# Golbstein/Keras-segmentation-deeplab-v3.1

Measured on AMD Instinct MI355X. Metric: images/sec fwd+bwd, 512x512 MobileNetV2 OS=16, 21 classes, higher is better.
Workload: dtype f32; 1 GPU; Deeplabv3(backbone='mobilenetv2', input_shape=(512,512,3), classes=21, OS=16) head=deeplab: fwd + sparse-xent loss + bwd + Adam, BN batch mode, dropout 0.1; global_batch=128, per_gpu_batch=128, parallelism=dp1, hipgraph=True, matrix_math=f32, dist_strict=False, backward_fork=False

## Files before the change

### keras-segmentation-deeplab-v3.1_amd/csrc/dwconv.hip

```cpp
#include "common.h"

#pragma clang fp contract(on)
#include <type_traits>
#include <stdlib.h>

namespace {

__device__ __forceinline__ f32x4 ld4_su(const float *base, unsigned byte_off) {
  return ld4(reinterpret_cast<const float *>(reinterpret_cast<const char *>(base) + byte_off));
}
__device__ __forceinline__ void st4_nt_su(float *base, unsigned byte_off, f32x4 v) {
  st4_nt(reinterpret_cast<float *>(reinterpret_cast<char *>(base) + byte_off), v);
}

struct DwGeom {
  int N, H, W, C, stride, rate, pad_t, pad_l, Ho, Wo;
  int prows;
};

struct DwMarch {
  int H, W, C, r, nchunk, TK, nxseg, nphase, ppb, nslab, ny, N;
  int prows;
  int fast;
};
// ... 313 lines not shown
    };
    if (ph.k0 < ph.k1) dw_walk<R>(ph, allact, ph.ke, group);
    if (!ph.bot_halo && ph.k0 < ph.k1) {
      float *orow = yn + (size_t)(a + (ph.k1 - 1) * r) * W * C;
      if (act_a) { st4_nt_su(orow, osa, aA); s1 += aA; s2 += aA * aA; }
      if (act_b) { st4_nt_su(orow, osb, bA); s1 += bA; s2 += bA * bA; }
    }
  }
  dw_store_stats(part, dw_tile_row(M, tile), M.N * M.ny * M.nxseg, M.prows, C, c, s1, s2, red);
}

template <bool SXK, bool ADDK>
__global__ __launch_bounds__(256, 2) void dw_march_bwd(
    const float *__restrict__ g, const float *__restrict__ yraw, const float *__restrict__ cA,
    const float *__restrict__ cB, const float *__restrict__ cC, const float *__restrict__ x,
    const float *__restrict__ sc, const float *__restrict__ sh, int act, const float *__restrict__ w,
    float *__restrict__ dx, const float *__restrict__ dx_add, const float *__restrict__ xmean,
    const float *__restrict__ xinvstd, float *__restrict__ dpart, float *__restrict__ wpart, DwMarch M,
    const float *__restrict__ sx) {
  __shared__ float red[4 * 8 * 36];
  const int tid = threadIdx.x, cq = tid & 7, pl = tid >> 3;
  DwTile tile;
  if (!dw_tile(M, tile)) return;
  const int H = M.H, W = M.W, C = M.C, r = M.r;
  const int xs = tile.xs, slab = tile.slab, n = tile.n;
  const int c = slab * 32 + cq * 4;
  const int xx = xs * 32 + pl;
  const bool active = (c < C) && (xx < W);

  const DwChan cn = dw_chan(c, C, w, sc, sh, cA, cB, cC, dpart != nullptr, xmean, xinvstd);
  const bool xl_ok = (xx - r >= 0), xr_ok = (xx + r < W);
  const int cc = min(c, C - 4), xc = min(xx, W - 1), xlc = min(max(xx - r, 0), W - 1), xrc = min(xx + r, W - 1);
  const size_t nimg = (size_t)n * H * W * C;
  const unsigned om = 4u * (unsigned)(xc * C + cc), ol = 4u * (unsigned)(xlc * C + cc), orr = 4u * (unsigned)(xrc * C + cc);
  const unsigned oo = 4u * (unsigned)(xx * C + c);
  const bool allact = M.fast && (slab * 32 + 32 <= C) && (xs * 32 + 32 <= W);
  f32x4 dwv[9];
#pragma unroll
  for (int i = 0; i < 9; i++) dwv[i] = splat4(0.f);
  f32x4 s1 = splat4(0.f), s2 = splat4(0.f);
  for (int pi = 0; pi < M.ppb; ++pi) {
    DwPhase ph;
    if (!dw_phase(M, tile.pc, pi, ph)) break;
    const int a = ph.a;
    const float *yr = dw_yr(cA, yraw, g);
    auto rowoff = [&](int k) -> size_t { return nimg + (size_t)(a + min(max(k, 0), ph.Kc) * r) * W * C; };

    auto ld_dd1 = [&](size_t row, unsigned off) -> f32x4 { return dw_dy(cn, ld4_su(g + row, off), ld4_su(yr + row, off)); };
    auto ld_dd = [&](int k, f32x4 &l, f32x4 &m, f32x4 &rr) {
      const bool rok = active && k >= 0 && k < ph.Ka;
      const size_t row = rowoff(k);
      const f32x4 vm = ld_dd1(row, om), vl = ld_dd1(row, ol), vr = ld_dd1(row, orr);
      m = vm * splat4(rok ? 1.f : 0.f);
      l = vl * splat4((rok && xl_ok) ? 1.f : 0.f);
      rr = vr * splat4((rok && xr_ok) ? 1.f : 0.f);
    };
    auto ld_e = [&](int k, f32x4 &raw, bool &ok) {
      ok = active && k >= 0 && k < ph.Ka;
      raw = ld4_su(x + rowoff(k), om);
    };
    auto eact = [&](f32x4 raw, bool ok) -> f32x4 {
      const f32x4 v = dl3_act4(cn.s * raw + cn.t, act);
      return v * splat4(ok ? 1.f : 0.f);
    };

    f32x4 accA = splat4(0.f), accB = splat4(0.f);

    if (ph.k0 < ph.k1) {
      constexpr int R = 2;
      f32x4 e_prev = splat4(0.f), e_cur, e_next;
      bool ok_prev = false, ok_cur, ok_next;
      ld_e(ph.ks, e_cur, ok_cur);
      ld_e(ph.ks + 1, e_next, ok_next);
      auto group = [&](int kg, auto fastc) __attribute__((always_inline)) {
        constexpr bool FAST = decltype(fastc)::value, SXC = SXK, ADDC = ADDK;
        f32x4 l[R], m[R], rr[R], e_new[R], sxv[R], addv[R];
        bool ok_new[R];
#pragma unroll
        for (int j = 0; j < R; j++) {
          if constexpr (FAST) {
            const size_t row = nimg + (size_t)(a + (kg + j) * r) * W * C;
            m[j] = ld_dd1(row, om);
            l[j] = ld_dd1(row, ol) * splat4(xl_ok ? 1.f : 0.f);
            rr[j] = ld_dd1(row, orr) * splat4(xr_ok ? 1.f : 0.f);
            ld_e(kg + j + 2, e_new[j], ok_new[j]);
            const size_t orow = nimg + (size_t)(a + (kg + j - 1) * r) * W * C;
            if constexpr (SXC) sxv[j] = ld4_su(sx + orow, om);
            if constexpr (ADDC) addv[j] = ld4_su(dx_add + orow, om);
          } else {
            ld_dd((kg + j <= ph.ke) ? kg + j : -1, l[j], m[j], rr[j]);
            ld_e(kg + j + 2, e_new[j], ok_new[j]);
            const size_t orow = rowoff(kg + j - 1);
            if constexpr (SXC) sxv[j] = ld4_su(sx + orow, om);
            if constexpr (ADDC) addv[j] = ld4_su(dx_add + orow, om);
          }
        }
#pragma unroll
        for (int j = 0; j < R; j++) {
          const int k = kg + j;
          const bool kv = FAST || k <= ph.ke;
          if (FAST || (k >= ph.k0 && k < ph.k1)) {
            f32x4 ea0 = eact(e_prev, ok_prev), ea1 = eact(e_cur, ok_cur), ea2 = eact(e_next, ok_next);
            dwv[0] += ea0 * rr[j]; dwv[1] += ea0 * m[j]; dwv[2] += ea0 * l[j];
            dwv[3] += ea1 * rr[j]; dwv[4] += ea1 * m[j]; dwv[5] += ea1 * l[j];
            dwv[6] += ea2 * rr[j]; dwv[7] += ea2 * m[j]; dwv[8] += ea2 * l[j];
          }
          f32x4 h0 = cn.wv[0] * rr[j] + cn.wv[1] * m[j] + cn.wv[2] * l[j];
          f32x4 h1 = cn.wv[3] * rr[j] + cn.wv[4] * m[j] + cn.wv[5] * l[j];
          f32x4 h2 = cn.wv[6] * rr[j] + cn.wv[7] * m[j] + cn.wv[8] * l[j];
          f32x4 out = accA + h0;
          if constexpr (FAST) {
            out = out * dl3_mask4(cn.s * e_prev + cn.t, act);
            if constexpr (ADDC) out += addv[j];
            st4_nt_su(dx + nimg + (size_t)(a + (k - 1) * r) * W * C, oo, out);
            s1 += out;
            s2 += out * (((SXC ? sxv[j] : e_prev) - cn.mu) * cn.is);
            accA = accB + h1;
            accB = h2;
            e_prev = e_cur; ok_prev = ok_cur;
            e_cur = e_next; ok_cur = ok_next;
            e_next = e_new[j]; ok_next = ok_new[j];
          } else {
            if (dx && active && kv && k - 1 >= ph.k0 && k - 1 < ph.k1) {
              out = out * dl3_mask4(cn.s * e_prev + cn.t, act);
              if constexpr (ADDC) out += addv[j];
              st4_nt_su(dx + nimg + (size_t)(a + (k - 1) * r) * W * C, oo, out);
              s1 += out;
              s2 += out * (((SXC ? sxv[j] : e_prev) - cn.mu) * cn.is);
            }
            accA = kv ? accB + h1 : accA;
            accB = kv ? h2 : accB;
            e_prev = kv ? e_cur : e_prev; ok_prev = kv ? ok_cur : ok_prev;
            e_cur = kv ? e_next : e_cur; ok_cur = kv ? ok_next : ok_cur;
            e_next = kv ? e_new[j] : e_next; ok_next = kv ? ok_new[j] : ok_next;
          }
        }
      };
      dw_walk<R>(ph, allact && dx, ph.k1 - 1, group);
      if (!ph.bot_halo && dx && active) {
        const size_t row = nimg + (size_t)(a + (ph.k1 - 1) * r) * W * C;
        f32x4 out = accA * dl3_mask4(cn.s * e_prev + cn.t, act);
        if constexpr (ADDK) out += ld4_su(dx_add + row, oo);
        st4_nt_su(dx + row, oo, out);
        s1 += out;
        s2 += out * (((SXK ? ld4_su(sx + row, oo) : e_prev) - cn.mu) * cn.is);
      }
    }
  }
  const int p = dw_tile_row(M, tile), written = M.N * M.ny * M.nxseg;
  dw_store_wgrad(wpart, p, written, M.prows, C, c, dwv, red);
  dw_store_stats(dpart, p, written, M.prows, C, c, s1, s2, red);
}

__global__ __launch_bounds__(256) void dw_gather_fwd(const float *__restrict__ x, const float *__restrict__ sc,
                                                     const float *__restrict__ sh, int act,
                                                     const float *__restrict__ w, float *__restrict__ y, DwGeom G,
                                                     float *__restrict__ part) {
  __shared__ float red[4 * 8 * 8];
  const int tid = threadIdx.x, cq = tid & 7, pl = tid >> 3;
  const int c = blockIdx.x * 32 + cq * 4;
  const bool cok = c < G.C;
  const DwChan cn = dw_chan(c, G.C, w, sc, sh);
  f32x4 s1 = splat4(0.f), s2 = splat4(0.f);
  const long NP = (long)G.N * G.Ho * G.Wo;
  for (long p = (long)blockIdx.y * 32 + pl; p < NP && cok; p += (long)gridDim.y * 32) {
    const int ox = (int)(p % G.Wo);
    const int oy = (int)((p / G.Wo) % G.Ho);
    const int n = (int)(p / ((long)G.Wo * G.Ho));
    f32x4 acc = splat4(0.f);
    f32x4 tap[9];
    float okf[9];
#pragma unroll
    for (int i = 0; i < 3; i++) {
      const int iy = oy * G.stride - G.pad_t + i * G.rate;
      const int iyc = min(max(iy, 0), G.H - 1);
#pragma unroll
      for (int j = 0; j < 3; j++) {
        const int ix = ox * G.stride - G.pad_l + j * G.rate;
        const int ixc = min(max(ix, 0), G.W - 1);
        okf[i * 3 + j] = (iy == iyc && ix == ixc) ? 1.f : 0.f;
        tap[i * 3 + j] = ld4(x + (((size_t)n * G.H + iyc) * G.W + ixc) * G.C + c);
      }
    }
#pragma unroll
    for (int q = 0; q < 9; q++) acc += (cn.wv[q] * splat4(okf[q])) * dl3_act4(cn.s * tap[q] + cn.t, act);
    st4_nt(y + (size_t)p * G.C + c, acc);
    s1 += acc;
    s2 += acc * acc;
  }
  dw_store_stats(part, blockIdx.y, gridDim.y, G.prows, G.C, c, s1, s2, red);
}

__global__ __launch_bounds__(256) void dw_gather_bwd(
    const float *__restrict__ g, const float *__restrict__ yraw, const float *__restrict__ cA,
    const float *__restrict__ cB, const float *__restrict__ cC, const float *__restrict__ x,
    const float *__restrict__ sc, const float *__restrict__ sh, int act, const float *__restrict__ w,
    float *__restrict__ dx, const float *__restrict__ dx_add, const float *__restrict__ xmean,
    const float *__restrict__ xinvstd, float *__restrict__ dpart, float *__restrict__ wpart, DwGeom G) {
  __shared__ float red[4 * 8 * 36];
  const int tid = threadIdx.x, cq = tid & 7, pl = tid >> 3;
  const int c = blockIdx.x * 32 + cq * 4;
  const bool cok = c < G.C;
  const DwChan cn = dw_chan(c, G.C, w, sc, sh, cA, cB, cC, dpart != nullptr, xmean, xinvstd);
  f32x4 dwv[9];
#pragma unroll
  for (int i = 0; i < 9; i++) dwv[i] = splat4(0.f);
  f32x4 s1 = splat4(0.f), s2 = splat4(0.f);
  const long NP = (long)G.N * G.H * G.W;
  for (long p = (long)blockIdx.y * 32 + pl; p < NP && cok; p += (long)gridDim.y * 32) {
    const int ix = (int)(p % G.W);
    const int iy = (int)((p / G.W) % G.H);
    const int n = (int)(p / ((long)G.W * G.H));
    const f32x4 eraw = ld4(x + (size_t)p * G.C + c);
    const f32x4 z = cn.s * eraw + cn.t;
    const f32x4 ea = dl3_act4(z, act);
    f32x4 acc = splat4(0.f);
    const float *yr = dw_yr(cA, yraw, g);
    f32x4 tg[9], ty_[9];
    float okf[9];
#pragma unroll
    for (int i = 0; i < 3; i++) {
      const int ty = iy + G.pad_t - i * G.rate;
      const int oy = max(ty, 0) / G.stride;
      const bool yok = ty >= 0 && (ty % G.stride) == 0 && oy < G.Ho;
      const int oyc = min(oy, G.Ho - 1);
#pragma unroll
      for (int j = 0; j < 3; j++) {
        const int tx = ix + G.pad_l - j * G.rate;
        const int ox = max(tx, 0) / G.stride;
        const bool xok = tx >= 0 && (tx % G.stride) == 0 && ox < G.Wo;
        const int oxc = min(ox, G.Wo - 1);
        const size_t off = (((size_t)n * G.Ho + oyc) * G.Wo + oxc) * G.C + c;
        okf[i * 3 + j] = (yok && xok) ? 1.f : 0.f;
        tg[i * 3 + j] = ld4(g + off);
        ty_[i * 3 + j] = ld4(yr + off);
      }
    }
#pragma unroll
    for (int q = 0; q < 9; q++) {
      const f32x4 dd = dw_dy(cn, tg[q], ty_[q]) * splat4(okf[q]);
      acc += dd * cn.wv[q];
      dwv[q] += ea * dd;
    }
    if (dx) {
      f32x4 out = acc * dl3_mask4(z, act);
      if (dx_add) out += ld4(dx_add + (size_t)p * G.C + c);
      st4_nt(dx + (size_t)p * G.C + c, out);
      s1 += out;
      s2 += out * ((eraw - cn.mu) * cn.is);
    }
  }
  dw_store_wgrad(wpart, blockIdx.y, gridDim.y, G.prows, G.C, c, dwv, red);
  dw_store_stats(dpart, blockIdx.y, gridDim.y, G.prows, G.C, c, s1, s2, red);
}

__global__ __launch_bounds__(256) void dw_s2_bwd(
    const float *__restrict__ g, const float *__restrict__ yraw, const float *__restrict__ cA,
    const float *__restrict__ cB, const float *__restrict__ cC, const float *__restrict__ x,
    const float *__restrict__ sc, const float *__restrict__ sh, int act, const float *__restrict__ w,
    float *__restrict__ dx, const float *__restrict__ dx_add, const float *__restrict__ xmean,
    const float *__restrict__ xinvstd, float *__restrict__ dpart, float *__restrict__ wpart, DwGeom G) {
  __shared__ float red[4 * 8 * 36];
  const int tid = threadIdx.x, cq = tid & 7, pl = tid >> 3;
  const int c = blockIdx.x * 32 + cq * 4;
  const bool cok = c < G.C;
  const int cc = min(c, G.C - 4);
  const DwChan cn = dw_chan(c, G.C, w, sc, sh, cA, cB, cC, dpart != nullptr, xmean, xinvstd);
  const float *yr = dw_yr(cA, yraw, g);
  f32x4 dwv[9];
#pragma unroll
  for (int i = 0; i < 9; i++) dwv[i] = splat4(0.f);
  f32x4 s1 = splat4(0.f), s2 = splat4(0.f);
  const int A = (G.H + G.pad_t + 1) / 2, Bn = (G.W + G.pad_l + 1) / 2;
  const long NB = (long)G.N * A * Bn;
  for (long q = (long)blockIdx.y * 32 + pl; q < NB; q += (long)gridDim.y * 32) {
    const int b = (int)(q % Bn), a = (int)((q / Bn) % A), n = (int)(q / ((long)Bn * A));
    const int iy0 = 2 * a - G.pad_t, ix0 = 2 * b - G.pad_l;
    f32x4 dd[2][2];
#pragma unroll
    for (int i = 0; i < 2; i++)
#pragma unroll
      for (int j = 0; j < 2; j++) {
        const int oy = a - i, ox = b - j;
        const int oyc = min(max(oy, 0), G.Ho - 1), oxc = min(max(ox, 0), G.Wo - 1);
        const float ok = (cok && oy == oyc && ox == oxc) ? 1.f : 0.f;
        const size_t off = (((size_t)n * G.Ho + oyc) * G.Wo + oxc) * G.C + cc;
        dd[i][j] = dw_dy(cn, ld4(g + off), ld4(yr + off)) * splat4(ok);
      }
    f32x4 xr[2][2], ad[2][2];
    float pok[2][2];
    size_t poff[2][2];
#pragma unroll
    for (int i = 0; i < 2; i++)
#pragma unroll
      for (int j = 0; j < 2; j++) {
        const int iy = iy0 + i, ix = ix0 + j;
        const int iyc = min(max(iy, 0), G.H - 1), ixc = min(max(ix, 0), G.W - 1);
        pok[i][j] = (cok && iy == iyc && ix == ixc) ? 1.f : 0.f;
        poff[i][j] = (((size_t)n * G.H + iyc) * G.W + ixc) * G.C + cc;
        xr[i][j] = ld4(x + poff[i][j]);
        ad[i][j] = dx_add ? ld4(dx_add + poff[i][j]) : splat4(0.f);
      }
    f32x4 acc[2][2];
    acc[0][0] = cn.wv[0] * dd[0][0] + cn.wv[6] * dd[1][0] + cn.wv[2] * dd[0][1] + cn.wv[8] * dd[1][1];
    acc[0][1] = cn.wv[1] * dd[0][0] + cn.wv[7] * dd[1][0];
    acc[1][0] = cn.wv[3] * dd[0][0] + cn.wv[5] * dd[0][1];
    acc[1][1] = cn.wv[4] * dd[0][0];
    f32x4 ea[2][2];
#pragma unroll
    for (int i = 0; i < 2; i++)
#pragma unroll
      for (int j = 0; j < 2; j++) ea[i][j] = dl3_act4(cn.s * xr[i][j] + cn.t, act) * splat4(pok[i][j]);
    dwv[0] += ea[0][0] * dd[0][0]; dwv[6] += ea[0][0] * dd[1][0]; dwv[2] += ea[0][0] * dd[0][1]; dwv[8] += ea[0][0] * dd[1][1];
    dwv[1] += ea[0][1] * dd[0][0]; dwv[7] += ea[0][1] * dd[1][0];
    dwv[3] += ea[1][0] * dd[0][0]; dwv[5] += ea[1][0] * dd[0][1];
    dwv[4] += ea[1][1] * dd[0][0];
    if (dx) {
#pragma unroll
      for (int i = 0; i < 2; i++)
#pragma unroll
        for (int j = 0; j < 2; j++) {
          f32x4 out = acc[i][j] * dl3_mask4(cn.s * xr[i][j] + cn.t, act) + ad[i][j];
          if (pok[i][j] != 0.f) {
            st4_nt(dx + poff[i][j], out);
            s1 += out;
            s2 += out * ((xr[i][j] - cn.mu) * cn.is);
          }
        }
    }
  }
  dw_store_wgrad(wpart, blockIdx.y, gridDim.y, G.prows, G.C, c, dwv, red);
  dw_store_stats(dpart, blockIdx.y, gridDim.y, G.prows, G.C, c, s1, s2, red);
}

struct DwPlan {
  int impl;
  int nslab, nxseg, nphase, nchunk, TK;
  int ppb, ny;
  int two;
  int PB;
  int P;
};

// ... 188 lines not shown
```

### keras-segmentation-deeplab-v3.1_amd/csrc/pwfused.hip

```cpp
#include <stdlib.h>

#include <type_traits>

#include "common.h"

namespace {

struct FusedArgs {
  const float *x; int ldx; const float *xs, *xt; int x_act;
  const float *g; int ldg; const float *y; int ldy; const float *cA, *cB, *cC;
  const float *wT;
  float *slab;
  float *dx; int lddx;
  const float *add; int ldadd;
  const float *sx; int ldsx; const float *mean, *invstd;
  float *part;
  int M, K, N, Mper;
};

constexpr int FMS = 32;

template <int KB, int NB, bool AUX>
__global__ __launch_bounds__(256, (KB * NB == 5 || AUX) ? 2 : 4) void pw_bwd_fused_kernel(FusedArgs P) {
  constexpr int KP = KB * 32, NP = NB * 32;
  constexpr int LDX = KP + 4, LDD = NP + 4, LDW = KP;
  constexpr int NBLK = KB * NB;
  constexpr int WB = (NBLK + 3) / 4;
  constexpr int XB = (KB + 3) / 4;
  __shared__ float Xr[FMS * LDX];
  __shared__ float Ds[FMS * LDD];
  __shared__ float Sx[AUX ? FMS * LDX : 1];
  __shared__ float Ad[AUX ? FMS * LDX : 1];
  __shared__ float Wl[NP * LDW];
  __shared__ float cfx[2 * KP];
  __shared__ float cfd[3 * NP];

  const int tid = threadIdx.x, lane = tid & 63, wave = tid >> 6;
  const int l31 = lane & 31, lhi = lane >> 5;
  const int bz = blockIdx.x;
  const int mbeg = bz * P.Mper, mend = min(P.M, mbeg + P.Mper);
  const bool two = (P.cA != nullptr);
  const bool sep = AUX && P.sx != nullptr && P.sx != P.x;
  const float hi = (P.x_act == DL3_ACT_RELU6) ? 6.f : __builtin_inff();

  for (int i = tid; i < KP; i += 256) {
    const int k = min(i, P.K - 1);
    cfx[i] = P.xs ? P.xs[k] : 1.f;
    cfx[KP + i] = P.xs ? P.xt[k] : 0.f;
  }
  for (int i = tid; i < NP; i += 256) {
    const int n = min(i, P.N - 1);
    cfd[i] = two ? P.cA[n] : 1.f;
    cfd[NP + i] = two ? P.cB[n] : 0.f;
    cfd[2 * NP + i] = two ? P.cC[n] : 0.f;
  }
  for (int i = tid; i < NP * KP; i += 256) {
    const int n = i / KP, k = i % KP;
    Wl[n * LDW + k] = (n < P.N && k < P.K) ? P.wT[(size_t)n * P.K + k] : 0.f;
  }

  f32x16 accw[WB];
#pragma unroll
  for (int b = 0; b < WB; b++)
#pragma unroll
    for (int r = 0; r < 16; r++) accw[b][r] = 0.f;
  float st1[XB], st2[XB];
#pragma unroll
  for (int b = 0; b < XB; b++) st1[b] = st2[b] = 0.f;

  f32x4 rx[KB], rg[NB], ry[NB], rs[AUX ? KB : 1], ra[AUX ? KB : 1];
  auto load_regs = [&](int m0) {
#pragma unroll
    for (int i = 0; i < KB; i++) {
      const int idx = tid + 256 * i;
      const int mr = idx / (KP / 4), kq = idx % (KP / 4);
      const int row = min(m0 + mr, P.M - 1), k = min(kq * 4, P.K - 4);
      rx[i] = ld4(P.x + (size_t)row * P.ldx + k);
      if constexpr (AUX) {
        if (sep) rs[i] = ld4(P.sx + (size_t)row * P.ldsx + k);
        if (P.add) ra[i] = ld4(P.add + (size_t)row * P.ldadd + k);
      }
    }
#pragma unroll
    for (int i = 0; i < NB; i++) {
      const int idx = tid + 256 * i;
      const int mr = idx / (NP / 4), nq = idx % (NP / 4);
      const int row = min(m0 + mr, P.M - 1), n = min(nq * 4, P.N - 4);
      rg[i] = ld4(P.g + (size_t)row * P.ldg + n);
      if (two) ry[i] = ld4(P.y + (size_t)row * P.ldy + n);
    }
  };
  auto store_lds = [&](int m0) {
#pragma unroll
    for (int i = 0; i < KB; i++) {
      const int idx = tid + 256 * i;
      const int mr = idx / (KP / 4), kq = idx % (KP / 4);
      st4(&Xr[mr * LDX + kq * 4], rx[i]);
      if constexpr (AUX) {
        if (sep) st4(&Sx[mr * LDX + kq * 4], rs[i]);
        if (P.add) st4(&Ad[mr * LDX + kq * 4], ra[i]);
      }
    }
#pragma unroll
    for (int i = 0; i < NB; i++) {
      const int idx = tid + 256 * i;
      const int mr = idx / (NP / 4), nq = idx % (NP / 4);
      const bool ok = (m0 + mr) < mend && nq * 4 < P.N;
      f32x4 v = ld4(cfd + nq * 4) * rg[i] + ld4(cfd + 2 * NP + nq * 4);
      if (two) v += ld4(cfd + NP + nq * 4) * ry[i];
      if (!ok) v = splat4(0.f);
      st4(&Ds[mr * LDD + nq * 4], v);
    }
  };

  __syncthreads();
  if (mbeg < mend) load_regs(mbeg);
  for (int m0 = mbeg; m0 < mend; m0 += FMS) {
    store_lds(m0);
    __syncthreads();
    if (m0 + FMS < mend) load_regs(m0 + FMS);

#pragma unroll
    for (int b = 0; b < WB; b++) {
      const int blk = wave + 4 * b;
      if (blk < NBLK) {
        const int kb = blk / NB, nb = blk % NB;
        const float sk = cfx[kb * 32 + l31], tk = cfx[KP + kb * 32 + l31];
#pragma unroll
        for (int s = 0; s < FMS / 2; s++) {
          const float a = dl3_act(sk * Xr[(2 * s + lhi) * LDX + kb * 32 + l31] + tk, P.x_act);
          const float bb = Ds[(2 * s + lhi) * LDD + nb * 32 + l31];
          accw[b] = __builtin_amdgcn_mfma_f32_32x32x2f32(a, bb, accw[b], 0, 0, 0);
        }
      }
    }
#pragma unroll
    for (int kx = 0; kx < XB; kx++) {
      const int kbx = 4 * kx + (3 - wave);
      if (kbx < KB) {
        f32x16 acc;
#pragma unroll
        for (int r = 0; r < 16; r++) acc[r] = 0.f;
#pragma unroll 8
        for (int s = 0; s < NP / 2; s++) {
          const float a = Ds[l31 * LDD + 2 * s + lhi];
          const float bb = Wl[(2 * s + lhi) * LDW + kbx * 32 + l31];
          acc = __builtin_amdgcn_mfma_f32_32x32x2f32(a, bb, acc, 0, 0, 0);
        }
        const int col = kbx * 32 + l31;
        const bool cok = col < P.K;
        const float sc = cfx[col], tc = cfx[KP + col];
        const float mu = (P.part && cok) ? P.mean[col] : 0.f, is = (P.part && cok) ? P.invstd[col] : 0.f;
#pragma unroll
        for (int r = 0; r < 16; r++) {
          const int rl = (r & 3) + 8 * (r >> 2) + 4 * lhi;
          const int row = m0 + rl;
          const float raw = Xr[rl * LDX + col];
          float v = acc[r];
          if (P.x_act != DL3_ACT_NONE) {
            const float z = sc * raw + tc;
            v = (z > 0.f && z < hi) ? v : 0.f;
          }
          float xh = raw;
          if constexpr (AUX) {
            if (P.add) v += Ad[rl * LDX + col];
            if (sep) xh = Sx[rl * LDX + col];
          }
          if (cok && row < mend) {
            __builtin_nontemporal_store(v, &P.dx[(size_t)row * P.lddx + col]);
            st1[kx] += v;
            st2[kx] += v * ((xh - mu) * is);
          }
        }
// ... 12 lines not shown
#pragma unroll
      for (int r = 0; r < 16; r++) {
        const int krow = kb * 32 + (r & 3) + 8 * (r >> 2) + 4 * lhi;
        if (krow < P.K && col < P.N) out[(size_t)krow * P.N + col] = accw[b][r];
      }
    }
  }
  if (P.part) {
#pragma unroll
    for (int kx = 0; kx < XB; kx++) {
      const int kbx = 4 * kx + (3 - wave);
      if (kbx < KB) {
        const float a1 = st1[kx] + __shfl_xor(st1[kx], 32, 64), a2 = st2[kx] + __shfl_xor(st2[kx], 32, 64);
        const int col = kbx * 32 + l31;
        if (lhi == 0 && col < P.K) {
          P.part[((size_t)bz * P.K + col) * 2 + 0] = a1;
          P.part[((size_t)bz * P.K + col) * 2 + 1] = a2;
        }
      }
    }
  }
}


struct FusedSlices { int lo[4], n[4], maxn; };

constexpr int fused_dw_blocks(int nblk, int w) { return nblk > w ? (nblk - w + 3) / 4 : 0; }

constexpr FusedSlices fused_slices(int KB, int NB) {
  FusedSlices s{};
  const int nblk = KB * NB, TS = 16 * NB, split = 4 / KB;
  int load[4] = {0, 0, 0, 0};
  for (int w = 0; w < 4; w++) { load[w] = 16 * fused_dw_blocks(nblk, w); s.n[w] = 0; s.lo[w] = 0; }
  for (int g = 0; g < KB; g++) {
    for (int t = 0; t < TS; t++) {
      int best = g;
      for (int p = 1; p < split; p++) {
        const int w = g + KB * p;
        if (load[w] <= load[best]) best = w;
      }
      s.n[best]++;
      load[best]++;
    }
    int lo = 0;
    for (int p = 0; p < split; p++) {
      const int w = g + KB * p;
      s.lo[w] = lo;
      lo += s.n[w];
    }
  }
  s.maxn = 0;
  for (int w = 0; w < 4; w++) s.maxn = s.n[w] > s.maxn ? s.n[w] : s.maxn;
  return s;
}

constexpr int cmax(int a, int b) { return a > b ? a : b; }

template <int KB, int NB, bool AUX>
struct Fused2 {
  static constexpr int KP = KB * 32, NP = NB * 32;
  static constexpr int LDX = KP + 4, LDD = NP + 4;
  static constexpr int NBLK = KB * NB;
  static constexpr int WB = (NBLK + 3) / 4;
  static constexpr int SPLIT = KB <= 2 ? 4 / KB : 1;
  static constexpr int XB = SPLIT > 1 ? 1 : (KB + 3) / 4;
  static constexpr int RPW = 16 / SPLIT;
  static constexpr FusedSlices SL = fused_slices(KB <= 2 ? KB : 1, NB);
  static constexpr int NWB = SPLIT > 1 ? SL.maxn : 1;
  static constexpr int LDW = KP;
  static constexpr int O_X = 0;
  static constexpr int O_D = O_X + FMS * LDX;
  static constexpr int O_S = O_D + FMS * LDD;
  static constexpr int O_A = O_S + (AUX ? FMS * LDX : 0);
  static constexpr int O_W = O_A + (AUX ? FMS * LDX : 0);
  static constexpr int O_CX = O_W + (SPLIT > 1 ? 0 : NP * LDW);
  static constexpr int O_CD = O_CX + 2 * KP;
  static constexpr int O_P = O_CD + 3 * NP;
  static constexpr int O_R = O_P + (SPLIT > 1 ? 4 * 1024 : 0);
  static constexpr int TOTAL = O_R + (SPLIT > 1 ? 256 : 0);
};

template <int KB, int NB, bool AUX, int OC>
__global__ __launch_bounds__(256, OC) void pw_bwd_fused2_kernel(FusedArgs P) {
  using C = Fused2<KB, NB, AUX>;
  constexpr int KP = C::KP, NP = C::NP, LDX = C::LDX, LDD = C::LDD, LDW = C::LDW, NBLK = C::NBLK;
  constexpr int SPLIT = C::SPLIT, XB = C::XB, WB = C::WB, NWB = C::NWB;
  __shared__ float smem[C::TOTAL];
  float *const Xr = smem + C::O_X, *const Ds = smem + C::O_D, *const Sx = smem + C::O_S, *const Ad = smem + C::O_A;
  float *const Wl = smem + C::O_W, *const cfx = smem + C::O_CX, *const cfd = smem + C::O_CD;
  float *const Pp = smem + C::O_P, *const red = smem + C::O_R;

  const int tid = threadIdx.x, lane = tid & 63;
  const int wave = __builtin_amdgcn_readfirstlane(tid >> 6);
  const int l31 = lane & 31, lhi = lane >> 5;
  const int bz = blockIdx.x;
  const int mbeg = bz * P.Mper, mend = min(P.M, mbeg + P.Mper);
  const bool two = (P.cA != nullptr);
  const bool sep = AUX && P.sx != nullptr && P.sx != P.x;
  const float hi = (P.x_act == DL3_ACT_RELU6) ? 6.f : __builtin_inff();

  for (int i = tid; i < KP; i += 256) {
    const int k = min(i, P.K - 1);
    cfx[i] = P.xs ? P.xs[k] : 1.f;
    cfx[KP + i] = P.xs ? P.xt[k] : 0.f;
  }
  for (int i = tid; i < NP; i += 256) {
    const int n = min(i, P.N - 1);
    cfd[i] = two ? P.cA[n] : 1.f;
    cfd[NP + i] = two ? P.cB[n] : 0.f;
    cfd[2 * NP + i] = two ? P.cC[n] : 0.f;
  }

  const int klast = P.K - 32 * (KB - 1);
  int x_kbx[XB], x_col[XB], x_lo = 0, x_n = NP / 2, x_part = 0;
  if constexpr (SPLIT > 1) {
    x_kbx[0] = wave % KB;
    x_part = wave / KB;
    x_lo = wave == 0 ? C::SL.lo[0] : wave == 1 ? C::SL.lo[1] : wave == 2 ? C::SL.lo[2] : C::SL.lo[3];
    x_n = wave == 0 ? C::SL.n[0] : wave == 1 ? C::SL.n[1] : wave == 2 ? C::SL.n[2] : C::SL.n[3];
  } else {
#pragma unroll
    for (int kx = 0; kx < XB; kx++) x_kbx[kx] = 4 * kx + (3 - wave);
  }
#pragma unroll
  for (int kx = 0; kx < XB; kx++) x_col[kx] = x_kbx[kx] * 32 + (x_kbx[kx] == KB - 1 ? l31 % klast : l31);
  float x_sc[XB], x_tc[XB], x_mu[XB], x_is[XB];
  float wb[NWB];
  if constexpr (SPLIT > 1) {
#pragma unroll
    for (int s = 0; s < NWB; s++) {
      const int n = 2 * (x_lo + s) + lhi;
      const bool ok = s < x_n && n < P.N;
      const float v = P.wT[(size_t)min(n, P.N - 1) * P.K + x_col[0]];
      wb[s] = ok ? v : 0.f;
    }
  } else {
    wb[0] = 0.f;
    for (int i = tid; i < NP * KP; i += 256) {
      const int n = i / KP, k = i % KP;
      Wl[n * LDW + k] = (n < P.N && k < P.K) ? P.wT[(size_t)n * P.K + k] : 0.f;
    }
  }

  f32x16 accw[WB];
#pragma unroll
  for (int b = 0; b < WB; b++)
#pragma unroll
    for (int r = 0; r < 16; r++) accw[b][r] = 0.f;
  float st1[XB], st2[XB];
#pragma unroll
  for (int b = 0; b < XB; b++) st1[b] = st2[b] = 0.f;

  f32x4 rx[KB], rg[NB], ry[NB], rs[AUX ? KB : 1], ra[AUX ? KB : 1];
  auto load_regs = [&](int m0) {
#pragma unroll
    for (int i = 0; i < KB; i++) {
      const int idx = tid + 256 * i;
      const int mr = idx / (KP / 4), kq = idx % (KP / 4);
      const int row = min(m0 + mr, P.M - 1), k = min(kq * 4, P.K - 4);
      rx[i] = ld4(P.x + (size_t)row * P.ldx + k);
      if constexpr (AUX) {
        if (sep) rs[i] = ld4(P.sx + (size_t)row * P.ldsx + k);
        if (P.add) ra[i] = ld4(P.add + (size_t)row * P.ldadd + k);
      }
    }
#pragma unroll
    for (int i = 0; i < NB; i++) {
      const int idx = tid + 256 * i;
      const int mr = idx / (NP / 4), nq = idx % (NP / 4);
      const int row = min(m0 + mr, P.M - 1), n = min(nq * 4, P.N - 4);
      rg[i] = ld4(P.g + (size_t)row * P.ldg + n);
      if (two) ry[i] = ld4(P.y + (size_t)row * P.ldy + n);
    }
  };
  auto store_lds = [&](int m0) {
#pragma unroll
    for (int i = 0; i < KB; i++) {
      const int idx = tid + 256 * i;
      const int mr = idx / (KP / 4), kq = idx % (KP / 4);
      st4(&Xr[mr * LDX + kq * 4], rx[i]);
      if constexpr (AUX) {
        if (sep) st4(&Sx[mr * LDX + kq * 4], rs[i]);
        if (P.add) st4(&Ad[mr * LDX + kq * 4], ra[i]);
      }
    }
#pragma unroll
    for (int i = 0; i < NB; i++) {
      const int idx = tid + 256 * i;
      const int mr = idx / (NP / 4), nq = idx % (NP / 4);
      const bool ok = (m0 + mr) < mend && nq * 4 < P.N;
      f32x4 v = ld4(cfd + nq * 4) * rg[i] + ld4(cfd + 2 * NP + nq * 4);
      if (two) v += ld4(cfd + NP + nq * 4) * ry[i];
      if (!ok) v = splat4(0.f);
      st4(&Ds[mr * LDD + nq * 4], v);
    }
  };

  auto finish = [&](auto fullc, float v, int m0, int rl, int col, bool own, float sc, float tc, float mu, float is,
                    float &s1, float &s2) {
    constexpr bool FULL = decltype(fullc)::value;
    const int row = m0 + rl;
    const float raw = Xr[rl * LDX + col];
    if (P.x_act != DL3_ACT_NONE) {
      const float z = sc * raw + tc;
      v = (z > 0.f && z < hi) ? v : 0.f;
    }
    float xh = raw;
    if constexpr (AUX) {
      if (P.add) v += Ad[rl * LDX + col];
      if (sep) xh = Sx[rl * LDX + col];
    }
    if constexpr (FULL) {
      __builtin_nontemporal_store(v, &P.dx[(size_t)row * P.lddx + col]);
      s1 += own ? v : 0.f;
      s2 += own ? v * ((xh - mu) * is) : 0.f;
    } else {
      if (own && row < mend) {
        __builtin_nontemporal_store(v, &P.dx[(size_t)row * P.lddx + col]);
        s1 += v;
        s2 += v * ((xh - mu) * is);
      }
    }
  };

  auto stage = [&](auto fullc, int m0) {
#pragma unroll
    for (int b = 0; b < WB; b++) {
      const int blk = wave + 4 * b;
      if (blk < NBLK) {
        const int kb = blk / NB, nb = blk % NB;
        const float sk = cfx[kb * 32 + l31], tk = cfx[KP + kb * 32 + l31];
#pragma unroll 4
        for (int s = 0; s < FMS / 2; s++) {
          const float a = dl3_act(sk * Xr[(2 * s + lhi) * LDX + kb * 32 + l31] + tk, P.x_act);
          const float bb = Ds[(2 * s + lhi) * LDD + nb * 32 + l31];
          accw[b] = __builtin_amdgcn_mfma_f32_32x32x2f32(a, bb, accw[b], 0, 0, 0);
        }
      }
    }

    if constexpr (SPLIT > 1) {
      f32x16 acc;
#pragma unroll
      for (int r = 0; r < 16; r++) acc[r] = 0.f;
      const float *dq = Ds + l31 * LDD + 2 * x_lo + lhi;
#pragma unroll
      for (int s = 0; s < NWB; s++)
        if (s < x_n) acc = __builtin_amdgcn_mfma_f32_32x32x2f32(dq[2 * s], wb[s], acc, 0, 0, 0);
      float *pp = Pp + wave * 1024 + lane;
#pragma unroll
      for (int r = 0; r < 16; r++) pp[r * 64] = acc[r];
      __syncthreads();
      const int kbx = x_kbx[0], col = x_col[0];
      const float *pq = Pp + kbx * 1024 + lane;
      const bool own = kbx * 32 + l31 < P.K;
      const float sc = x_sc[0], tc = x_tc[0], mu = x_mu[0], is = x_is[0];
#pragma unroll
      for (int rr = 0; rr < C::RPW; rr++) {
        const int r = x_part * C::RPW + rr;
        float v = pq[r * 64];
#pragma unroll
        for (int p = 1; p < SPLIT; p++) v += pq[p * KB * 1024 + r * 64];
        finish(fullc, v, m0, (r & 3) + 8 * (r >> 2) + 4 * lhi, col, own, sc, tc, mu, is, st1[0], st2[0]);
      }
    } else {
#pragma unroll
      for (int kx = 0; kx < XB; kx++) {
        const int kbx = x_kbx[kx];
        if (kbx < KB) {
          f32x16 acc;
#pragma unroll
          for (int r = 0; r < 16; r++) acc[r] = 0.f;
          const int col = x_col[kx];
#pragma unroll 8
          for (int s = 0; s < NP / 2; s++) {
            const float a = Ds[l31 * LDD + 2 * s + lhi];
            const float bb = Wl[(2 * s + lhi) * LDW + col];
            acc = __builtin_amdgcn_mfma_f32_32x32x2f32(a, bb, acc, 0, 0, 0);
          }
          const bool own = kbx * 32 + l31 < P.K;
          const float sc = x_sc[kx], tc = x_tc[kx], mu = x_mu[kx], is = x_is[kx];
#pragma unroll
          for (int r = 0; r < 16; r++)
            finish(fullc, acc[r], m0, (r & 3) + 8 * (r >> 2) + 4 * lhi, col, own, sc, tc, mu, is, st1[kx], st2[kx]);
        }
      }
    }
  };

  __syncthreads();
#pragma unroll
  for (int kx = 0; kx < XB; kx++) {
    const int col = min(x_col[kx], KP - 1);
    x_sc[kx] = cfx[col];
    x_tc[kx] = cfx[KP + col];
    x_mu[kx] = P.part ? P.mean[min(col, P.K - 1)] : 0.f;
    x_is[kx] = P.part ? P.invstd[min(col, P.K - 1)] : 0.f;
  }
  const int mfull = mbeg + ((mend > mbeg ? mend - mbeg : 0) / FMS) * FMS;
  if (mbeg < mend) load_regs(mbeg);
  auto whole_stage = [&](int m0) {
    store_lds(m0);
    __syncthreads();
    if (m0 + FMS < mend) load_regs(m0 + FMS);
    stage(std::true_type{}, m0);
    __syncthreads();
  };
  for (int m0 = mbeg; m0 < mfull; m0 += FMS) whole_stage(m0);
  if (mfull < mend) {
    store_lds(mfull);
    __syncthreads();
    stage(std::false_type{}, mfull);
    __syncthreads();
  }

  float *out = P.slab + (size_t)bz * P.K * P.N;
#pragma unroll
  for (int b = 0; b < WB; b++) {
    const int blk = wave + 4 * b;
    if (blk < NBLK) {
      const int kb = blk / NB, nb = blk % NB;
      const int col = nb * 32 + l31;
#pragma unroll
      for (int r = 0; r < 16; r++) {
        const int krow = kb * 32 + (r & 3) + 8 * (r >> 2) + 4 * lhi;
        if (krow < P.K && col < P.N) out[(size_t)krow * P.N + col] = accw[b][r];
      }
    }
  }
  if (P.part) {
    if constexpr (SPLIT > 1) {
      const float a1 = st1[0] + __shfl_xor(st1[0], 32, 64), a2 = st2[0] + __shfl_xor(st2[0], 32, 64);
      if (lhi == 0) {
        red[(wave * 32 + l31) * 2 + 0] = a1;
        red[(wave * 32 + l31) * 2 + 1] = a2;
      }
      __syncthreads();
      const int kbx = x_kbx[0], col = kbx * 32 + l31;
      if (x_part == 0 && lhi == 0 && col < P.K) {
        float b1 = red[(kbx * 32 + l31) * 2 + 0], b2 = red[(kbx * 32 + l31) * 2 + 1];
#pragma unroll
        for (int p = 1; p < SPLIT; p++) {
          b1 += red[((kbx + KB * p) * 32 + l31) * 2 + 0];
          b2 += red[((kbx + KB * p) * 32 + l31) * 2 + 1];
        }
        P.part[((size_t)bz * P.K + col) * 2 + 0] = b1;
        P.part[((size_t)bz * P.K + col) * 2 + 1] = b2;
      }
    } else {
#pragma unroll
      for (int kx = 0; kx < XB; kx++) {
        const int kbx = x_kbx[kx];
        if (kbx < KB) {
          const float a1 = st1[kx] + __shfl_xor(st1[kx], 32, 64), a2 = st2[kx] + __shfl_xor(st2[kx], 32, 64);
          const int col = kbx * 32 + l31;
          if (lhi == 0 && col < P.K) {
            P.part[((size_t)bz * P.K + col) * 2 + 0] = a1;
            P.part[((size_t)bz * P.K + col) * 2 + 1] = a2;
          }
        }
      }
    }
  }
}

int fused_env(const char *name) {
  const char *e = getenv(name);
  return e ? atoi(e) : -1;
}
int fused_version() { return fused_env("DL3_FUSED_V") == 1 ? 1 : 2; }

int fused_rows_per_wg(int M) {
  long want = 2048;
  long stages = dl3_cdiv(M, FMS);
  {
    long cap = (long)M / 512;
    if (cap < 512) cap = 512;
    if (want > cap) want = cap;
  }
  if (want > stages) want = stages;
  return (int)(dl3_cdiv((int)stages, (int)want) * FMS);
}

inline bool al16(const void *p) { return (((uintptr_t)p) & 15) == 0; }

}

extern "C" int dl3_reduce_partials(const float *partial, int P, int n, float *out, void *stream);

extern "C" int dl3_pwconv_bwd_fused_supported(int M, int K, int N) {
  if (M <= 0 || K < 4 || N < 4 || K % 4 || N % 4) return 0;
  if (dl3_cdiv(K, 32) * dl3_cdiv(N, 32) > (fused_version() == 1 ? 5 : 6)) return 0;
  return K <= 64 ? 2 : 1;
}

extern "C" int dl3_pwconv_bwd_fused_splits(int M, int K, int N) {
  if (!dl3_pwconv_bwd_fused_supported(M, K, N)) return 0;
  return dl3_cdiv(M, fused_rows_per_wg(M));
}

extern "C" size_t dl3_pwconv_bwd_fused_workspace(int M, int K, int N) {
  return (size_t)dl3_pwconv_bwd_fused_splits(M, K, N) * K * N * sizeof(float);
}

extern "C" int dl3_pwconv_bwd_fused(const float *x, int ldx, const float *in_scale, const float *in_shift, int in_act,
                                    const float *g, int ldg, const float *yraw, int ldyraw, const float *cA,
                                    const float *cB, const float *cC, const float *wT, float *dw, float *dx, int lddx,
                                    const float *dx_add, int ldadd, const float *stat_x, int ldstatx,
                                    const float *x_mean, const float *x_invstd, float *dstat_partial, int M, int K,
                                    int N, void *workspace, size_t workspace_bytes, void *stream) {
  DL3_CHECK_ARG(M > 0 && K > 0 && N > 0, "pwconv_bwd_fused: non-positive dimension");
  DL3_UNSUPPORTED(!dl3_pwconv_bwd_fused_supported(M, K, N),
                  "pwconv_bwd_fused: K=%d, N=%d must be multiples of 4 with ceil(K/32)*ceil(N/32) <= 6", K, N);
  DL3_CHECK_ARG(x && g && wT && dx && workspace, "pwconv_bwd_fused: null pointer");
  DL3_CHECK_ARG(!cA || (yraw && cB && cC), "pwconv_bwd_fused: cA needs yraw, cB, cC");
  DL3_CHECK_ARG((in_scale == nullptr) == (in_shift == nullptr), "pwconv_bwd_fused: scale/shift must come together");
  DL3_CHECK_ARG(!dstat_partial || (stat_x && x_mean && x_invstd), "pwconv_bwd_fused: dstat needs stat_x, x_mean, x_invstd");
  DL3_CHECK_ARG(ldx >= K && ldx % 4 == 0 && al16(x) && ldg >= N && ldg % 4 == 0 && al16(g) &&
                    (!cA || (ldyraw >= N && ldyraw % 4 == 0 && al16(yraw))) && lddx >= K,
                "pwconv_bwd_fused: operands must be 16-byte aligned with leading dimensions that are multiples of 4");
  if (workspace_bytes < dl3_pwconv_bwd_fused_workspace(M, K, N)) {
    dl3_set_error("pwconv_bwd_fused: workspace %zu < %zu bytes", workspace_bytes, dl3_pwconv_bwd_fused_workspace(M, K, N));
    return DL3_EWORKSPACE;
  }
  FusedArgs A{};
  A.x = x; A.ldx = ldx; A.xs = in_scale; A.xt = in_shift; A.x_act = in_act;
  A.g = g; A.ldg = ldg; A.y = cA ? yraw : nullptr; A.ldy = ldyraw; A.cA = cA; A.cB = cB; A.cC = cC;
  A.wT = wT; A.slab = (float *)workspace; A.dx = dx; A.lddx = lddx; A.add = dx_add; A.ldadd = ldadd;
  A.sx = dstat_partial ? stat_x : nullptr; A.ldsx = ldstatx; A.mean = x_mean; A.invstd = x_invstd;
  A.part = dstat_partial;
  A.M = M; A.K = K; A.N = N; A.Mper = fused_rows_per_wg(M);
  const int S = dl3_cdiv(M, A.Mper);
  hipStream_t st = (hipStream_t)stream;
  const int kb = dl3_cdiv(K, 32), nb = dl3_cdiv(N, 32);
  const bool aux = dx_add != nullptr || (A.sx != nullptr && A.sx != x);
  DL3_UNSUPPORTED(aux && kb > 2, "pwconv_bwd_fused: a residual addend / sums against another tensor need K <= 64 (K=%d)", K);
  DL3_CHECK_ARG(!aux || ((!dx_add || (ldadd % 4 == 0 && al16(dx_add))) && (!A.sx || (ldstatx % 4 == 0 && al16(A.sx)))),
                "pwconv_bwd_fused: dx_add / stat_x must be 16-byte aligned with leading dimensions that are multiples of 4");
  if (fused_version() == 1) {
#define DL3_FUSED(KB_, NB_, AUX_) \
  if (kb == KB_ && nb == NB_ && aux == AUX_) \
    hipLaunchKernelGGL((pw_bwd_fused_kernel<KB_, NB_, AUX_>), dim3(S), dim3(256), 0, st, A)
  DL3_FUSED(1, 1, false); DL3_FUSED(1, 2, false); DL3_FUSED(1, 3, false); DL3_FUSED(1, 4, false); DL3_FUSED(1, 5, false);
  DL3_FUSED(2, 1, false); DL3_FUSED(3, 1, false); DL3_FUSED(4, 1, false); DL3_FUSED(5, 1, false); DL3_FUSED(2, 2, false);
  DL3_FUSED(1, 1, true); DL3_FUSED(1, 2, true); DL3_FUSED(1, 3, true); DL3_FUSED(1, 4, true); DL3_FUSED(1, 5, true);
  DL3_FUSED(2, 1, true); DL3_FUSED(2, 2, true);
#undef DL3_FUSED
  } else {
#define DL3_FUSED(KB_, NB_, AUX_, OC_) \
  if (kb == KB_ && nb == NB_ && aux == AUX_) \
    hipLaunchKernelGGL((pw_bwd_fused2_kernel<KB_, NB_, AUX_, OC_>), dim3(S), dim3(256), 0, st, A)
  DL3_FUSED(1, 1, false, 4); DL3_FUSED(1, 2, false, 4); DL3_FUSED(1, 3, false, 3); DL3_FUSED(1, 4, false, 3);
  DL3_FUSED(1, 5, false, 2); DL3_FUSED(1, 6, false, 2);
  DL3_FUSED(2, 1, false, 4); DL3_FUSED(2, 2, false, 3); DL3_FUSED(2, 3, false, 2);
  DL3_FUSED(3, 1, false, 4); DL3_FUSED(4, 1, false, 4); DL3_FUSED(5, 1, false, 2); DL3_FUSED(6, 1, false, 2);
  DL3_FUSED(3, 2, false, 3);
  DL3_FUSED(1, 1, true, 3); DL3_FUSED(1, 2, true, 3); DL3_FUSED(1, 3, true, 3); DL3_FUSED(1, 4, true, 3);
  DL3_FUSED(1, 5, true, 2); DL3_FUSED(1, 6, true, 2); DL3_FUSED(2, 1, true, 3); DL3_FUSED(2, 2, true, 3);
  DL3_FUSED(2, 3, true, 2);
#undef DL3_FUSED
  }
  DL3_LAUNCH_CHECK("pwconv_bwd_fused");
  if (!dw) return DL3_OK;
  return dl3_reduce_partials(A.slab, S, K * N, dw, stream);
}
```

Before: 1346 img/s.

## Remap dw gather blocks across XCDs and slim pw bwd fused register use

The depthwise gather forward kernel now remaps its linear block index so that consecutive logical blocks are grouped per XCD (blocks are dealt round-robin across 8 chiplets), which should improve L2 locality for neighbouring channel slabs and pixel blocks. In the fused pointwise backward kernel, a LEAN path for KB>=5 recomputes addresses as a scalar base plus a 32-bit byte offset and hoists per-lane offsets, with asm barriers to stop the compiler from rematerializing values. This is meant to cut VGPR pressure. The activation check is also made branchless, and the 5x1 instantiation's occupancy template parameter rises from 2 to 3. Risks include register spills if the occupancy target is too high, and 32-bit offset overflow on large tensors.

```diff
diff --git a/keras-segmentation-deeplab-v3.1_amd/csrc/dwconv.hip b/keras-segmentation-deeplab-v3.1_amd/csrc/dwconv.hip
--- a/keras-segmentation-deeplab-v3.1_amd/csrc/dwconv.hip
+++ b/keras-segmentation-deeplab-v3.1_amd/csrc/dwconv.hip
@@ -489,18 +489,27 @@
   dw_store_stats(dpart, p, written, M.prows, C, c, s1, s2, red);
 }
 
+struct DwBlock { int slab, pb; };
+__device__ __forceinline__ DwBlock dw_gather_block() {
+  const int nwg = gridDim.x * gridDim.y, b = blockIdx.y * gridDim.x + blockIdx.x;
+  const int xq = nwg >> 3, xr = nwg & 7, xcd = b & 7;
+  const int v = (xcd < xr ? xcd * (xq + 1) : xr * (xq + 1) + (xcd - xr) * xq) + (b >> 3);
+  return DwBlock{__builtin_amdgcn_readfirstlane(v % (int)gridDim.x), __builtin_amdgcn_readfirstlane(v / (int)gridDim.x)};
+}
+
 __global__ __launch_bounds__(256) void dw_gather_fwd(const float *__restrict__ x, const float *__restrict__ sc,
                                                      const float *__restrict__ sh, int act,
                                                      const float *__restrict__ w, float *__restrict__ y, DwGeom G,
                                                      float *__restrict__ part) {
   __shared__ float red[4 * 8 * 8];
   const int tid = threadIdx.x, cq = tid & 7, pl = tid >> 3;
-  const int c = blockIdx.x * 32 + cq * 4;
+  const DwBlock wg = dw_gather_block();
+  const int c = wg.slab * 32 + cq * 4;
   const bool cok = c < G.C;
   const DwChan cn = dw_chan(c, G.C, w, sc, sh);
   f32x4 s1 = splat4(0.f), s2 = splat4(0.f);
   const long NP = (long)G.N * G.Ho * G.Wo;
-  for (long p = (long)blockIdx.y * 32 + pl; p < NP && cok; p += (long)gridDim.y * 32) {
+  for (long p = (long)wg.pb * 32 + pl; p < NP && cok; p += (long)gridDim.y * 32) {
     const int ox = (int)(p % G.Wo);
     const int oy = (int)((p / G.Wo) % G.Ho);
     const int n = (int)(p / ((long)G.Wo * G.Ho));
@@ -525,7 +534,7 @@
     s1 += acc;
     s2 += acc * acc;
   }
-  dw_store_stats(part, blockIdx.y, gridDim.y, G.prows, G.C, c, s1, s2, red);
+  dw_store_stats(part, wg.pb, gridDim.y, G.prows, G.C, c, s1, s2, red);
 }
 
 __global__ __launch_bounds__(256) void dw_gather_bwd(
diff --git a/keras-segmentation-deeplab-v3.1_amd/csrc/pwfused.hip b/keras-segmentation-deeplab-v3.1_amd/csrc/pwfused.hip
--- a/keras-segmentation-deeplab-v3.1_amd/csrc/pwfused.hip
+++ b/keras-segmentation-deeplab-v3.1_amd/csrc/pwfused.hip
@@ -19,6 +19,10 @@
 };
 
 constexpr int FMS = 32;
+
+__device__ __forceinline__ f32x4 ld4_su(const float *base, unsigned byte_off) {
+  return ld4(reinterpret_cast<const float *>(reinterpret_cast<const char *>(base) + byte_off));
+}
 
 template <int KB, int NB, bool AUX>
 __global__ __launch_bounds__(256, (KB * NB == 5 || AUX) ? 2 : 4) void pw_bwd_fused_kernel(FusedArgs P) {
@@ -337,25 +341,32 @@
   for (int b = 0; b < XB; b++) st1[b] = st2[b] = 0.f;
 
   f32x4 rx[KB], rg[NB], ry[NB], rs[AUX ? KB : 1], ra[AUX ? KB : 1];
+  constexpr bool LEAN = KB >= 5;
   auto load_regs = [&](int m0) {
+    int tl = tid;
+    if constexpr (LEAN) asm volatile("" : "+v"(tl));
+    auto row4 = [&](const float *p, int ld, int mr, int c) -> f32x4 {
+      if constexpr (LEAN) return ld4_su(p + (size_t)m0 * ld, 4u * (unsigned)(min(mr, P.M - 1 - m0) * ld + c));
+      else return ld4(p + (size_t)min(m0 + mr, P.M - 1) * ld + c);
+    };
 #pragma unroll
     for (int i = 0; i < KB; i++) {
-      const int idx = tid + 256 * i;
+      const int idx = tl + 256 * i;
       const int mr = idx / (KP / 4), kq = idx % (KP / 4);
-      const int row = min(m0 + mr, P.M - 1), k = min(kq * 4, P.K - 4);
-      rx[i] = ld4(P.x + (size_t)row * P.ldx + k);
+      const int k = min(kq * 4, P.K - 4);
+      rx[i] = row4(P.x, P.ldx, mr, k);
       if constexpr (AUX) {
-        if (sep) rs[i] = ld4(P.sx + (size_t)row * P.ldsx + k);
-        if (P.add) ra[i] = ld4(P.add + (size_t)row * P.ldadd + k);
+        if (sep) rs[i] = row4(P.sx, P.ldsx, mr, k);
+        if (P.add) ra[i] = row4(P.add, P.ldadd, mr, k);
       }
     }
 #pragma unroll
     for (int i = 0; i < NB; i++) {
-      const int idx = tid + 256 * i;
+      const int idx = tl + 256 * i;
       const int mr = idx / (NP / 4), nq = idx % (NP / 4);
-      const int row = min(m0 + mr, P.M - 1), n = min(nq * 4, P.N - 4);
-      rg[i] = ld4(P.g + (size_t)row * P.ldg + n);
-      if (two) ry[i] = ld4(P.y + (size_t)row * P.ldy + n);
+      const int n = min(nq * 4, P.N - 4);
+      rg[i] = row4(P.g, P.ldg, mr, n);
+      if (two) ry[i] = row4(P.y, P.ldy, mr, n);
     }
   };
   auto store_lds = [&](int m0) {
@@ -381,27 +392,41 @@
     }
   };
 
-  auto finish = [&](auto fullc, float v, int m0, int rl, int col, bool own, float sc, float tc, float mu, float is,
-                    float &s1, float &s2) {
+  const bool noact = (P.x_act == DL3_ACT_NONE);
+  auto lane_part = [&](int col, int &xl, unsigned &dl) {
+    if constexpr (LEAN) asm volatile("" : "+v"(col));
+    xl = 4 * lhi * LDX + col;
+    dl = 4u * (unsigned)(4 * lhi * P.lddx + col);
+  };
+  auto finish = [&](auto fullc, float v, int m0, int rs, int col, int xl, unsigned dl, bool own, float sc, float tc,
+                    float mu, float is, float &s1, float &s2) {
     constexpr bool FULL = decltype(fullc)::value;
-    const int row = m0 + rl;
-    const float raw = Xr[rl * LDX + col];
-    if (P.x_act != DL3_ACT_NONE) {
+    const int rl = rs + 4 * lhi, row = m0 + rl;
+    const int xi = LEAN ? rs * LDX + xl : rl * LDX + col;
+    float *const dq = LEAN ? reinterpret_cast<float *>(reinterpret_cast<char *>(P.dx + (size_t)(m0 + rs) * P.lddx) + dl)
+                           : &P.dx[(size_t)row * P.lddx + col];
+    const float raw = Xr[xi];
+    if constexpr (LEAN) {
       const float z = sc * raw + tc;
-      v = (z > 0.f && z < hi) ? v : 0.f;
+      v = (noact | ((z > 0.f) & (z < hi))) ? v : 0.f;
+    } else {
+      if (P.x_act != DL3_ACT_NONE) {
+        const float z = sc * raw + tc;
+        v = (z > 0.f && z < hi) ? v : 0.f;
+      }
     }
     float xh = raw;
     if constexpr (AUX) {
-      if (P.add) v += Ad[rl * LDX + col];
-      if (sep) xh = Sx[rl * LDX + col];
+      if (P.add) v += Ad[xi];
+      if (sep) xh = Sx[xi];
     }
     if constexpr (FULL) {
-      __builtin_nontemporal_store(v, &P.dx[(size_t)row * P.lddx + col]);
+      __builtin_nontemporal_store(v, dq);
       s1 += own ? v : 0.f;
       s2 += own ? v * ((xh - mu) * is) : 0.f;
     } else {
       if (own && row < mend) {
-        __builtin_nontemporal_store(v, &P.dx[(size_t)row * P.lddx + col]);
+        __builtin_nontemporal_store(v, dq);
         s1 += v;
         s2 += v * ((xh - mu) * is);
       }
@@ -437,6 +462,9 @@
       for (int r = 0; r < 16; r++) pp[r * 64] = acc[r];
       __syncthreads();
       const int kbx = x_kbx[0], col = x_col[0];
+      int xl;
+      unsigned dl;
+      lane_part(col, xl, dl);
       const float *pq = Pp + kbx * 1024 + lane;
       const bool own = kbx * 32 + l31 < P.K;
       const float sc = x_sc[0], tc = x_tc[0], mu = x_mu[0], is = x_is[0];
@@ -446,7 +474,7 @@
         float v = pq[r * 64];
 #pragma unroll
         for (int p = 1; p < SPLIT; p++) v += pq[p * KB * 1024 + r * 64];
-        finish(fullc, v, m0, (r & 3) + 8 * (r >> 2) + 4 * lhi, col, own, sc, tc, mu, is, st1[0], st2[0]);
+        finish(fullc, v, m0, (r & 3) + 8 * (r >> 2), col, xl, dl, own, sc, tc, mu, is, st1[0], st2[0]);
       }
     } else {
 #pragma unroll
@@ -465,9 +493,12 @@
           }
           const bool own = kbx * 32 + l31 < P.K;
           const float sc = x_sc[kx], tc = x_tc[kx], mu = x_mu[kx], is = x_is[kx];
+          int xl;
+          unsigned dl;
+          lane_part(col, xl, dl);
 #pragma unroll
           for (int r = 0; r < 16; r++)
-            finish(fullc, acc[r], m0, (r & 3) + 8 * (r >> 2) + 4 * lhi, col, own, sc, tc, mu, is, st1[kx], st2[kx]);
+            finish(fullc, acc[r], m0, (r & 3) + 8 * (r >> 2), col, xl, dl, own, sc, tc, mu, is, st1[kx], st2[kx]);
         }
       }
     }
@@ -638,7 +669,7 @@
   DL3_FUSED(1, 1, false, 4); DL3_FUSED(1, 2, false, 4); DL3_FUSED(1, 3, false, 3); DL3_FUSED(1, 4, false, 3);
   DL3_FUSED(1, 5, false, 2); DL3_FUSED(1, 6, false, 2);
   DL3_FUSED(2, 1, false, 4); DL3_FUSED(2, 2, false, 3); DL3_FUSED(2, 3, false, 2);
-  DL3_FUSED(3, 1, false, 4); DL3_FUSED(4, 1, false, 4); DL3_FUSED(5, 1, false, 2); DL3_FUSED(6, 1, false, 2);
+  DL3_FUSED(3, 1, false, 4); DL3_FUSED(4, 1, false, 4); DL3_FUSED(5, 1, false, 3); DL3_FUSED(6, 1, false, 2);
   DL3_FUSED(3, 2, false, 3);
   DL3_FUSED(1, 1, true, 3); DL3_FUSED(1, 2, true, 3); DL3_FUSED(1, 3, true, 3); DL3_FUSED(1, 4, true, 3);
   DL3_FUSED(1, 5, true, 2); DL3_FUSED(1, 6, true, 2); DL3_FUSED(2, 1, true, 3); DL3_FUSED(2, 2, true, 3);
```

Result: no change. 1346 img/s (-0.0%).
